# dotchen/LAV

Hardware: NVIDIA H100
Metric: agent_frames_per_s (higher is better)
Workload: dtype fp16 storage, fp32 accumulate (wgmma f16 / mma.sync f16; saturating stores)

## Files before the change

### include/lav_b200.h

```cpp
#ifndef LAV_B200_H
#define LAV_B200_H

#include <stddef.h>
#include <stdint.h>

#ifdef __cplusplus
extern "C" {
#endif

#define LAVB_ABI_VERSION 3

int lavb_abi_version(void);
const char* lavb_last_error(void);
int lavb_device_cc(void);

enum { LAVB_F32 = 0, LAVB_BF16 = 1, LAVB_F16 = 2 };
int lavb_h16_dtype(void);

int lavb_paint(const float* d_pts, int n, int pt_stride,
               const float* d_sem, int ncam, int c_in, int h, int w,
               long long s_cam, long long s_c, long long s_y, long long s_x,
               const float* h_cams, int mode,
               float* d_out, int out_stride, int out_col0, int copy_cols, void* stream);

// ... 115 lines not shown
int lavb_stack_job_poses(void* d_jobs, int b, int t, int gap, int keep, long long tick, double* d_ring_pose, const double* d_poses,
                         void* stream);

#define LAVB_VIEW_JET_ROWS 259
typedef struct lavb_view_config {
  double pixels_per_meter, cmd_thresh;
  unsigned char jet[LAVB_VIEW_JET_ROWS * 3];
} lavb_view_config;

size_t lavb_agent_view_scratch_bytes(int b);
int lavb_agent_view(const unsigned char* d_rgbs, const unsigned char* d_tels, const float* d_points, int b, long long p,
                    int point_stride, const void* d_bev, int bev_dtype, int bev_c, const long long* h_bev_strides, const float* d_plan,
                    const float* d_cast, const int* d_cmd, int t, const float* d_other_locs, const float* d_other_cmds, int k, int m,
                    const int* h_offsets, const double* h_boxes, int n_boxes, const int* h_box_offsets, const float* d_target,
                    const lavb_view_config* h_config, void* d_scratch, size_t scratch_bytes, unsigned char* d_out, void* stream);

size_t lavb_pillar_workspace_bytes(int batch, int nx, int ny);
int lavb_pillar_forward(const float* d_pts, int pt_stride, int d,
                        const long long* h_cloud_start, const int* h_cloud_count, int batch,
                        float min_x, float max_x, float min_y, float max_y, float ppm, int nx, int ny,
                        const float* d_w1, const float* d_s1, const float* d_t1, int h1,
                        const float* d_w2, const float* d_s2, const float* d_t2, int h2,
                        void* d_canvas, int canvas_dtype, void* d_workspace, void* stream);

size_t lavb_pillar_sorted_workspace_bytes(int batch, int nx, int ny, long long total_points);
int lavb_pillar_forward_sorted(const float* d_pts, int pt_stride, int d,
                               const long long* h_cloud_start, const int* h_cloud_count, int batch,
                               float min_x, float max_x, float min_y, float max_y, float ppm, int nx, int ny,
                               const float* d_w1, const float* d_s1, const float* d_t1, int h1,
                               const float* d_w2, const float* d_s2, const float* d_t2, int h2,
                               void* d_canvas, int out_mode, void* d_workspace, void* stream);

int lavb_pillar_decorate(const float* d_pts, int pt_stride, int d,
                         const long long* h_cloud_start, const int* h_cloud_count, int batch,
                         float min_x, float max_x, float min_y, float max_y, float ppm, int nx, int ny,
                         float* d_feat, int* d_cell, int* h_m, void* d_workspace, void* stream);
int lavb_pillar_scatter_max(const float* d_h, const int* d_cell, int m, int c, long long n_cells,
                            float* d_canvas, int* d_argmax, void* stream);
int lavb_pillar_scatter_max_bwd(const float* d_gcanvas, const int* d_argmax, const int* d_cell, int m, int c,
                                float* d_gh, void* stream);

typedef struct {
  const void* in; int in_dtype; int n, hin, win, cin, in_cstride, in_coff;
  void* out; int out_dtype; int hout, wout, cout, out_cstride, out_coff;
  int hog, wog;
  int in_sy, in_sx, out_sy, out_sx, out_oy, out_ox;
  int ntaps; int dy[16]; int dx[16];
  const float* w; const float* bias; const float* scale; const float* shift;
  const void* res; int res_dtype; int res_cstride, res_coff;
  int pre_relu, post_relu, sigmoid;
  int d2s_nout;
} lavb_conv_desc;
int lavb_conv_taps(const lavb_conv_desc* h_desc, void* stream);

int lavb_deconv3x3s2_small(const void* d_in, int dtype, int n, int h, int w, int in_cstride, int groups, int cin_g,
                           const float* d_w, const float* d_bias, const int* h_n_out, const int* h_sigmoid,
                           float* const* h_out_ptrs, void* stream);

int lavb_pool2_affine_relu(const void* d_in, int dtype, int n, int hin, int win, int c, int in_cstride, int in_coff,
                           const float* d_scale, const float* d_shift,
                           void* d_out, int out_cstride, int out_coff, void* stream);

int lavb_rgb_normalize(const void* d_rgb, int src_is_u8_nhwc, int n, int h, int w, void* d_out, int out_dtype,
                       void* stream);

int lavb_stem7x7s2_u8(const void* d_img, int batch, int ncam, int h, int cam_w, const void* d_w, const float* d_bias,
                      const float* h_mean, const float* h_std, void* d_out, void* stream);
int lavb_maxpool3x3s2_nhwc(const void* d_in, int n, int h, int w, int c, void* d_out, void* stream);

size_t lavb_det_peaks_workspace_bytes(int batch, int ncls);
int lavb_det_peaks(const float* d_center, const float* d_box, const float* d_ori, int batch, int h, int w, int ncls,
                   float min_score, int max_det, float* d_packed, void* d_workspace, void* stream);

int lavb_crop_bilinear(const void* d_feat, int dtype, int b, int h, int w, int c, const int* d_frame_idx,
                       const float* d_theta, int k, int crop, void* d_out, void* stream);
int lavb_crop_bilinear_u8(const uint8_t* d_map, int b, int c, int h, int w, const int* d_frame_idx, const float* d_theta,
                          int k, int crop, float* d_out, void* stream);
int lavb_crop_bilinear_bwd(const float* d_gout, int b, int h, int w, int c, const int* d_frame_idx, const float* d_theta,
                           int k, int crop, float* d_gfeat, void* stream);

int lavb_convert(const void* d_src, int src_dtype, void* d_dst, int dst_dtype, long long count, void* stream);

int lavb_conv_umma(const lavb_conv_desc* h_desc, void* stream);

int lavb_conv7x7s2_umma(const void* d_in, int n, int h, int w, int cin, const void* d_w, const float* d_bias, void* d_out,
                        void* stream);

int lavb_conv3x3_umma(const void* d_in, int n, int h, int w, int cin, int stride, const void* d_w, int cout, const float* d_bias,
                      const float* d_scale, const float* d_shift, int pre_relu, void* d_out, void* stream);

typedef struct lavb_conv_pair_desc {
  const void* in; void* out; const void* res;
  int n, h, w, c, dil, post_relu;
  const void* w1; const float* bias1;
  const void* w2; const float* shift2;
} lavb_conv_pair_desc;
int lavb_conv_pair_umma(const lavb_conv_pair_desc* h_desc, void* stream);
int lavb_conv_pair_set_trace(void* d_buf, int tiles_per_cta);

int lavb_erf_stem(const void* d_rgb_u8, int n, int h, int w, const float* h_w27x16, const float* h_scale16,
                  const float* h_shift16, void* d_out, int out_dtype, void* stream);

int lavb_erf_down16(const void* d_in, void* d_out, int n, int h, int w, const float* d_w9, const float* d_st, void* stream);

int lavb_erf_nb16(const void* d_in, void* d_out, int n, int h, int w, const float* d_w4, const float* d_st, void* stream);

int lavb_cast_gru(const float* d_embd, int n, const float* d_wih_t, const float* d_whh_t, const float* d_bih, const float* d_bhh,
                  const float* d_wmlp, const float* d_bmlp, int ncmd, int steps, float* d_out, void* stream);

#ifdef __cplusplus
}
#endif
#endif
```

### lav_b200/capi.py

```python
import ctypes as C
import os

_HERE = os.path.dirname(os.path.abspath(__file__))
LIB_PATH = os.path.join(_HERE, "_lib", "liblavb200.so")

F32, BF16, F16 = 0, 1, 2


class LavbError(RuntimeError):
    pass


class ConvDesc(C.Structure):
    _fields_ = [
        ("inp", C.c_void_p), ("in_dtype", C.c_int), ("n", C.c_int), ("hin", C.c_int), ("win", C.c_int), ("cin", C.c_int),
        ("in_cstride", C.c_int), ("in_coff", C.c_int),
        ("out", C.c_void_p), ("out_dtype", C.c_int), ("hout", C.c_int), ("wout", C.c_int), ("cout", C.c_int),
        ("out_cstride", C.c_int), ("out_coff", C.c_int),
        ("hog", C.c_int), ("wog", C.c_int),
        ("in_sy", C.c_int), ("in_sx", C.c_int), ("out_sy", C.c_int), ("out_sx", C.c_int), ("out_oy", C.c_int), ("out_ox", C.c_int),
        ("ntaps", C.c_int), ("dy", C.c_int * 16), ("dx", C.c_int * 16),
        ("w", C.c_void_p), ("bias", C.c_void_p), ("scale", C.c_void_p), ("shift", C.c_void_p),
        ("res", C.c_void_p), ("res_dtype", C.c_int), ("res_cstride", C.c_int), ("res_coff", C.c_int),
        ("pre_relu", C.c_int), ("post_relu", C.c_int), ("sigmoid", C.c_int), ("d2s_nout", C.c_int),
# ... 53 lines not shown
    "lavb_det_heatmaps": (C.c_int, [C.c_void_p, C.c_void_p, C.c_int, C.c_int, C.c_int, C.c_float, C.c_float, C.c_float, C.c_float,
                                    C.c_float, C.c_void_p, C.c_void_p, C.c_void_p, C.c_void_p]),
    "lavb_eval_batch": (C.c_int, [C.c_void_p, C.c_int, C.c_void_p, C.c_int, C.c_int, C.c_int, C.c_int, C.c_void_p, C.c_int,
                                  C.c_void_p, C.c_int, C.c_void_p, C.c_float, C.c_float, C.c_float, C.c_float, C.c_double,
                                  C.c_void_p, C.c_void_p, C.c_int, C.c_void_p, C.c_void_p, C.c_void_p, C.c_void_p, C.c_void_p,
                                  C.c_void_p]),
    "lavb_forecast_eval": (C.c_int, [C.c_void_p, C.c_void_p, C.c_void_p, C.c_void_p, C.c_int, C.c_int, C.c_int, C.c_void_p,
                                     C.c_void_p, C.c_void_p]),
    "lavb_det_forecast_match": (C.c_int, [C.c_void_p, C.c_int, C.c_int, C.c_int, C.c_void_p, C.c_int, C.c_void_p, C.c_void_p,
                                          C.c_void_p, C.c_void_p, C.c_void_p, C.c_void_p, C.c_int, C.c_int, C.c_float, C.c_float,
                                          C.c_float, C.c_float, C.c_double, C.c_void_p, C.c_void_p, C.c_void_p, C.c_void_p,
                                          C.c_void_p, C.c_void_p]),
    "lavb_det_box_eval": (C.c_int, [C.c_void_p, C.c_int, C.c_int, C.c_int, C.c_void_p, C.c_int, C.c_void_p, C.c_float, C.c_float,
                                    C.c_float, C.c_float, C.c_double, C.c_void_p, C.c_void_p, C.c_void_p, C.c_void_p, C.c_void_p,
                                    C.c_void_p]),
    "lavb_plan_safety": (C.c_int, [C.c_void_p, C.c_int, C.c_int, C.c_int, C.c_void_p, C.c_int, C.c_void_p, C.c_void_p, C.c_void_p,
                                   C.c_longlong, C.c_int, C.c_int, C.c_float, C.c_float, C.c_float, C.c_float, C.c_void_p,
                                   C.c_void_p]),
    "lavb_agent_control_state_bytes": (C.c_size_t, [C.c_int, C.c_int]),
    "lavb_agent_control": (C.c_int, [C.c_void_p, C.c_void_p, C.c_int, C.c_int, C.c_int, C.c_void_p, C.c_void_p, C.c_int, C.c_void_p,
                                     C.c_void_p, C.c_void_p, C.c_void_p, C.POINTER(ControlConfig), C.c_void_p, C.c_void_p,
                                     C.c_void_p, C.c_void_p]),
    "lavb_agent_control_dcmd": (C.c_int, [C.c_void_p, C.c_void_p, C.c_int, C.c_int, C.c_int, C.c_void_p, C.c_void_p, C.c_int,
                                          C.c_void_p, C.c_void_p, C.c_void_p, C.c_void_p, C.POINTER(ControlConfig), C.c_void_p,
                                          C.c_void_p, C.c_void_p, C.c_void_p]),
    "lavb_agent_nav_state_bytes": (C.c_size_t, []),
    "lavb_agent_nav_front": (C.c_int, [C.c_int, C.c_void_p, C.c_void_p, C.c_int, C.c_void_p, C.c_void_p, C.c_void_p, C.c_void_p,
                                       C.c_void_p, C.c_void_p, C.c_void_p, C.c_void_p, C.c_void_p]),
    "lavb_agent_nav_update": (C.c_int, [C.c_int, C.c_void_p, C.c_void_p, C.c_void_p, C.c_void_p, C.c_void_p, C.c_void_p]),
    "lavb_stack_job_poses": (C.c_int, [C.c_void_p, C.c_int, C.c_int, C.c_int, C.c_int, C.c_longlong, C.c_void_p, C.c_void_p,
                                       C.c_void_p]),
    "lavb_agent_view_scratch_bytes": (C.c_size_t, [C.c_int]),
    "lavb_agent_view": (C.c_int, [C.c_void_p, C.c_void_p, C.c_void_p, C.c_int, C.c_longlong, C.c_int, C.c_void_p, C.c_int, C.c_int,
                                  C.c_void_p, C.c_void_p, C.c_void_p, C.c_void_p, C.c_int, C.c_void_p, C.c_void_p, C.c_int, C.c_int,
                                  C.c_void_p, C.c_void_p, C.c_int, C.c_void_p, C.c_void_p, C.POINTER(ViewConfig), C.c_void_p,
                                  C.c_size_t, C.c_void_p, C.c_void_p]),
    "lavb_roof_filter": (C.c_int, [C.c_void_p, C.c_int, C.c_int, C.c_int, C.c_longlong, C.c_void_p, C.c_longlong, C.c_void_p, C.c_int,
                                   C.c_void_p]),
    "lavb_stack_sweep": (C.c_int, [C.c_void_p, C.c_int, C.c_int, C.c_void_p, C.c_float, C.c_float, C.c_int, C.c_int, C.c_int,
                                   C.c_void_p, C.c_void_p]),
    "lavb_pillar_workspace_bytes": (C.c_size_t, [C.c_int, C.c_int, C.c_int]),
    "lavb_pillar_forward": (C.c_int, [C.c_void_p, C.c_int, C.c_int, C.c_void_p, C.c_void_p, C.c_int,
                                      C.c_float, C.c_float, C.c_float, C.c_float, C.c_float, C.c_int, C.c_int,
                                      C.c_void_p, C.c_void_p, C.c_void_p, C.c_int, C.c_void_p, C.c_void_p, C.c_void_p, C.c_int,
                                      C.c_void_p, C.c_int, C.c_void_p, C.c_void_p]),
    "lavb_pillar_sorted_workspace_bytes": (C.c_size_t, [C.c_int, C.c_int, C.c_int, C.c_longlong]),
    "lavb_pillar_forward_sorted": (C.c_int, [C.c_void_p, C.c_int, C.c_int, C.c_void_p, C.c_void_p, C.c_int,
                                             C.c_float, C.c_float, C.c_float, C.c_float, C.c_float, C.c_int, C.c_int,
                                             C.c_void_p, C.c_void_p, C.c_void_p, C.c_int, C.c_void_p, C.c_void_p, C.c_void_p, C.c_int,
                                             C.c_void_p, C.c_int, C.c_void_p, C.c_void_p]),
    "lavb_pillar_decorate": (C.c_int, [C.c_void_p, C.c_int, C.c_int, C.c_void_p, C.c_void_p, C.c_int,
                                       C.c_float, C.c_float, C.c_float, C.c_float, C.c_float, C.c_int, C.c_int,
                                       C.c_void_p, C.c_void_p, C.c_void_p, C.c_void_p, C.c_void_p]),
    "lavb_pillar_scatter_max": (C.c_int, [C.c_void_p, C.c_void_p, C.c_int, C.c_int, C.c_longlong, C.c_void_p, C.c_void_p,
                                          C.c_void_p]),
    "lavb_pillar_scatter_max_bwd": (C.c_int, [C.c_void_p, C.c_void_p, C.c_void_p, C.c_int, C.c_int, C.c_void_p, C.c_void_p]),
    "lavb_conv_taps": (C.c_int, [C.POINTER(ConvDesc), C.c_void_p]),
    "lavb_pool2_affine_relu": (C.c_int, [C.c_void_p, C.c_int, C.c_int, C.c_int, C.c_int, C.c_int, C.c_int, C.c_int,
                                         C.c_void_p, C.c_void_p, C.c_void_p, C.c_int, C.c_int, C.c_void_p]),
    "lavb_rgb_normalize": (C.c_int, [C.c_void_p, C.c_int, C.c_int, C.c_int, C.c_int, C.c_void_p, C.c_int, C.c_void_p]),
    "lavb_convert": (C.c_int, [C.c_void_p, C.c_int, C.c_void_p, C.c_int, C.c_longlong, C.c_void_p]),
    "lavb_stem7x7s2_u8": (C.c_int, [C.c_void_p, C.c_int, C.c_int, C.c_int, C.c_int, C.c_void_p, C.c_void_p, C.c_void_p, C.c_void_p,
                                    C.c_void_p, C.c_void_p]),
    "lavb_erf_stem": (C.c_int, [C.c_void_p, C.c_int, C.c_int, C.c_int, C.c_void_p, C.c_void_p, C.c_void_p, C.c_void_p, C.c_int, C.c_void_p]),
    "lavb_erf_down16": (C.c_int, [C.c_void_p, C.c_void_p, C.c_int, C.c_int, C.c_int, C.c_void_p, C.c_void_p, C.c_void_p]),
    "lavb_erf_nb16": (C.c_int, [C.c_void_p, C.c_void_p, C.c_int, C.c_int, C.c_int, C.c_void_p, C.c_void_p, C.c_void_p]),
    "lavb_conv_pair_umma": (C.c_int, [C.c_void_p, C.c_void_p]),
    "lavb_maxpool3x3s2_nhwc": (C.c_int, [C.c_void_p, C.c_int, C.c_int, C.c_int, C.c_int, C.c_void_p, C.c_void_p]),
    "lavb_det_peaks_workspace_bytes": (C.c_size_t, [C.c_int, C.c_int]),
    "lavb_det_peaks": (C.c_int, [C.c_void_p, C.c_void_p, C.c_void_p, C.c_int, C.c_int, C.c_int, C.c_int, C.c_float, C.c_int,
                                 C.c_void_p, C.c_void_p, C.c_void_p]),
    "lavb_crop_bilinear": (C.c_int, [C.c_void_p, C.c_int, C.c_int, C.c_int, C.c_int, C.c_int, C.c_void_p, C.c_void_p, C.c_int,
                                     C.c_int, C.c_void_p, C.c_void_p]),
    "lavb_crop_bilinear_u8": (C.c_int, [C.c_void_p, C.c_int, C.c_int, C.c_int, C.c_int, C.c_void_p, C.c_void_p, C.c_int, C.c_int,
                                        C.c_void_p, C.c_void_p]),
    "lavb_cast_gru": (C.c_int, [C.c_void_p, C.c_int, C.c_void_p, C.c_void_p, C.c_void_p, C.c_void_p, C.c_void_p, C.c_void_p, C.c_int,
                                C.c_int, C.c_void_p, C.c_void_p]),
    "lavb_conv_pair_set_trace": (C.c_int, [C.c_void_p, C.c_int]),
    "lavb_crop_bilinear_bwd": (C.c_int, [C.c_void_p, C.c_int, C.c_int, C.c_int, C.c_int, C.c_void_p, C.c_void_p, C.c_int, C.c_int,
                                         C.c_void_p, C.c_void_p]),
    "lavb_deconv3x3s2_small": (C.c_int, [C.c_void_p, C.c_int, C.c_int, C.c_int, C.c_int, C.c_int, C.c_int, C.c_int, C.c_void_p,
                                         C.c_void_p, C.c_void_p, C.c_void_p, C.c_void_p, C.c_void_p]),
    "lavb_conv_umma": (C.c_int, [C.POINTER(ConvDesc), C.c_void_p]),
    "lavb_conv7x7s2_umma": (C.c_int, [C.c_void_p, C.c_int, C.c_int, C.c_int, C.c_int, C.c_void_p, C.c_void_p, C.c_void_p,
                                      C.c_void_p]),
    "lavb_conv3x3_umma": (C.c_int, [C.c_void_p, C.c_int, C.c_int, C.c_int, C.c_int, C.c_int, C.c_void_p, C.c_int, C.c_void_p,
                                    C.c_void_p, C.c_void_p, C.c_int, C.c_void_p, C.c_void_p]),
}

_lib = None


def exported_symbols():
    return sorted(_SIGS)


def lib():
    global _lib
    if _lib is None:
        if not os.path.exists(LIB_PATH):
            raise LavbError(f"{LIB_PATH} is missing — run `python -m lav_b200.build` (or __graft_entry__.build()); "
                            "lav_b200 has no CPU fallback")
        handle = C.CDLL(LIB_PATH)
        for name, (res, args) in _SIGS.items():
            fn = getattr(handle, name)
            fn.restype = res
            fn.argtypes = args
        if handle.lavb_abi_version() != 3:
            raise LavbError("liblavb200.so ABI version mismatch")
        _lib = handle
    return _lib


def h16_code():
    return lib().lavb_h16_dtype()


def check(code, what):
    if code != 0:
        raise LavbError(f"{what} failed ({code}): {lib().lavb_last_error().decode()}")
```

### lav_b200/csrc/conv_umma.cu

```cuda
#include "sm90.cuh"

namespace lavb {

constexpr int kTileH = 8, kTileW = 16, kBlockM = 128, kBlockK = 64;
constexpr int kABytes = kBlockM * kBlockK * 2;
constexpr int kMaxStages = 8;
constexpr int kMaxTaps = 16;
constexpr int kConvThreads = 288;

struct ConvArgs {
  int n, hog, wog, tiles_x, tiles_y, num_tiles;
  int hout, wout, cin, cout, kchunks, ntaps, stages;
  int in_sy, in_sx, out_sy, out_sx, out_oy, out_ox;
  int out_cstride, out_coff, out_is_f32, res_cstride, res_coff;
  int pre_bias, pre_relu, post_relu, sigmoid, d2s_nout, cout_store;
  int dy[kMaxTaps], dx[kMaxTaps];
  void* out; const h16* res;
  const float* bias; const float* scale; const float* shift;
};

using namespace sm90;

template <int kNC>
__global__ void __launch_bounds__(kConvThreads, kNC <= 4 ? 2 : 1) conv_umma_kernel(const __grid_constant__ CUtensorMap tmap_a,
                                                                                 const __grid_constant__ CUtensorMap tmap_b,
                                                                                 const __grid_constant__ ConvArgs p) {
  constexpr int kN = 32 * kNC;
  constexpr int kBBytes = kN * kBlockK * 2;
  constexpr int kStageBytes = kABytes + kBBytes;
  extern __shared__ uint8_t smem_raw[];
  const uint32_t base = (smem_u32(smem_raw) + 1023u) & ~1023u;
  uint8_t* gen = smem_raw + (base - smem_u32(smem_raw));
  const uint32_t ctrl = base + p.stages * kStageBytes;
  const uint32_t full_bar = ctrl, empty_bar = ctrl + 8 * kMaxStages;
  float* ep_bias = reinterpret_cast<float*>(gen + (ctrl - base) + 16 * kMaxStages);
  float* ep_st = ep_bias + 256;

  const int warp = threadIdx.x >> 5, lane = threadIdx.x & 31;
  if (threadIdx.x == 0) {
    asm volatile("prefetch.tensormap [%0];" ::"l"(reinterpret_cast<uint64_t>(&tmap_a)) : "memory");
    asm volatile("prefetch.tensormap [%0];" ::"l"(reinterpret_cast<uint64_t>(&tmap_b)) : "memory");
    for (int s = 0; s < p.stages; ++s) { mbar_init(full_bar + 8 * s, 1); mbar_init(empty_bar + 8 * s, 8); }
    asm volatile("fence.mbarrier_init.release.cluster;" ::: "memory");
  }
  for (int c = threadIdx.x; c < kN; c += blockDim.x) {
    const bool real = c < p.cout_store;
    const float b = (p.bias && real) ? __ldg(p.bias + c) : 0.f;
    const float sc = (p.scale && real) ? __ldg(p.scale + c) : 1.f;
    const float sh = (p.shift && real) ? __ldg(p.shift + c) : 0.f;
    ep_bias[c] = b;
    ep_st[2 * c] = sc;
    ep_st[2 * c + 1] = p.pre_bias ? sh : fmaf(b, sc, sh);
  }
  __syncthreads();
  const int nkb = p.ntaps * p.kchunks;
  const int tiles_per_img = p.tiles_x * p.tiles_y;

  if (warp == 8) {
    if (lane == 0) {
      int stage = 0; uint32_t phase = 0;
      for (int tile = blockIdx.x; tile < p.num_tiles; tile += gridDim.x) {
        const int img = tile / tiles_per_img, r = tile - img * tiles_per_img;
        const int y0 = (r / p.tiles_x) * kTileH * p.in_sy, x0 = (r % p.tiles_x) * kTileW * p.in_sx;
        for (int t = 0; t < p.ntaps; ++t) {
          for (int kc = 0; kc < p.kchunks; ++kc) {
            mbar_wait(empty_bar + 8 * stage, phase ^ 1);
            const uint32_t sa = base + stage * kStageBytes;
            mbar_expect_tx(full_bar + 8 * stage, kStageBytes);
            tma_load_4d(sa, &tmap_a, full_bar + 8 * stage, kc * kBlockK, x0 + p.dx[t], y0 + p.dy[t], img);
            tma_load_2d(sa + kABytes, &tmap_b, full_bar + 8 * stage, kc * kBlockK, t * kN);
            if (++stage == p.stages) { stage = 0; phase ^= 1; }
          }
        }
      }
    }
    return;
  }

  const int wg = warp >> 2;
  const float lo_pre = p.pre_relu ? 0.f : -INFINITY, lo_post = p.post_relu ? 0.f : -INFINITY;
  int stage = 0; uint32_t phase = 0;
  float acc[16 * kNC];
  for (int tile = blockIdx.x; tile < p.num_tiles; tile += gridDim.x) {
    int prev_stage = -1;
    for (int kb = 0; kb < nkb; ++kb) {
      mbar_wait(full_bar + 8 * stage, phase);
      const uint32_t sa = base + stage * kStageBytes;
      const uint64_t a_desc = sm90::desc_sw128(sa + wg * (kABytes / 2)), b_desc = sm90::desc_sw128(sa + kABytes);
      sm90::wgmma_fence();
#pragma unroll
      for (int k = 0; k < kBlockK / 16; ++k)
        sm90::wgmma<kN>(acc, a_desc + (uint64_t)(2 * k), b_desc + (uint64_t)(2 * k), (kb | k) ? 1u : 0u);
      sm90::wgmma_commit();
      sm90::wgmma_wait<1>();
      if (prev_stage >= 0 && lane == 0) mbar_arrive(empty_bar + 8 * prev_stage);
      prev_stage = stage;
      if (++stage == p.stages) { stage = 0; phase ^= 1; }
    }
    sm90::wgmma_wait<0>();
    sm90::acc_fence(acc);
    if (prev_stage >= 0 && lane == 0) mbar_arrive(empty_bar + 8 * prev_stage);

    const int c0 = 2 * (lane & 3), store_lim = p.cout_store - c0;
    const int img = tile / tiles_per_img, r = tile - img * tiles_per_img;
    const int gy = (r / p.tiles_x) * kTileH + 4 * wg + (warp & 3), oy = gy * p.out_sy + p.out_oy;
    if (!(gy < p.hog && oy < p.hout)) continue;
#pragma unroll
    for (int h = 0; h < 2; ++h) {
      const int gx = (r % p.tiles_x) * kTileW + (lane >> 2) + 8 * h, ox = gx * p.out_sx + p.out_ox;
      if (!(gx < p.wog && ox < p.wout)) continue;
      const long long pix = ((long long)img * p.hout + oy) * p.wout + ox;
      uint8_t* out_at = reinterpret_cast<uint8_t*>(p.out) + (pix * p.out_cstride + p.out_coff + c0) * (p.out_is_f32 ? 4 : 2);
      const h16* res_at = p.res ? p.res + pix * p.res_cstride + p.res_coff + c0 : nullptr;
      const float* bias_at = ep_bias + c0;
      const float* st_at = ep_st + 2 * c0;
#pragma unroll
      for (int j = 0; j < 4 * kNC; ++j) {
        const int g = 8 * j;
        float x0 = acc[4 * j + 2 * h], x1 = acc[4 * j + 2 * h + 1];
        if (p.pre_bias) { x0 += bias_at[g]; x1 += bias_at[g + 1]; }
        const float4 st = *reinterpret_cast<const float4*>(st_at + 2 * g);
        x0 = fmaf(fmaxf(x0, lo_pre), st.x, st.y);
        x1 = fmaf(fmaxf(x1, lo_pre), st.z, st.w);
        if (res_at) {
          const float2 rv = unpack_h16(__ldg(reinterpret_cast<const uint32_t*>(res_at + g)));
          x0 += rv.x; x1 += rv.y;
        }
        x0 = fmaxf(x0, lo_post); x1 = fmaxf(x1, lo_post);
        if (p.sigmoid) { x0 = 1.f / (1.f + expf(-x0)); x1 = 1.f / (1.f + expf(-x1)); }
        if (kNC == 1 && p.d2s_nout) {
          float* ob = reinterpret_cast<float*>(p.out);
          const int no = p.d2s_nout;
#pragma unroll
          for (int e = 0; e < 2; ++e) {
            const int q = g + c0 + e;
            if (q < 4 * no) {
              const int pos = q / no, k = q - pos * no;
              ob[(pix + (long long)(pos >> 1) * p.wout + (pos & 1)) * no + k] = e ? x1 : x0;
            }
          }
        } else if (g < store_lim) {
          if (p.out_is_f32)
            *reinterpret_cast<float2*>(out_at + 4 * g) = make_float2(x0, x1);
          else
            *reinterpret_cast<uint32_t*>(out_at + 2 * g) = pack_h16(x0, x1);
        }
      }
    }
  }
}

}

using namespace lavb;

extern "C" int lavb_conv_umma(const lavb_conv_desc* d, void* stream) {
  LAVB_CHECK_ARG(d != nullptr, "conv_umma: null descriptor");
  LAVB_CHECK_ARG(d->in_dtype == LAVB_H16, "conv_umma: input must be h16");
  LAVB_CHECK_ARG(d->out_dtype == LAVB_H16 || d->out_dtype == LAVB_F32, "conv_umma: bad output dtype");
  LAVB_CHECK_ARG(d->ntaps >= 1 && d->ntaps <= kMaxTaps, "conv_umma: ntaps must be 1..16");
  LAVB_CHECK_ARG(d->cin % 64 == 0 && d->cin > 0, "conv_umma: cin must be a multiple of 64 (got %d)", d->cin);
  LAVB_CHECK_ARG(d->cout % 8 == 0 && d->cout >= 8 && d->cout <= 256, "conv_umma: cout must be 8..256, multiple of 8 (got %d)", d->cout);
  const int cout_mma = (d->cout + 31) / 32 * 32;
  LAVB_CHECK_ARG(d->res == nullptr || cout_mma == d->cout, "conv_umma: residual needs cout %% 32 == 0");
  LAVB_CHECK_ARG(d->in_cstride % 8 == 0 && d->in_coff % 8 == 0 && d->in_coff + d->cin <= d->in_cstride, "conv_umma: input slice misaligned");
  LAVB_CHECK_ARG(d->out_cstride % 8 == 0 && d->out_coff % 8 == 0 && d->out_coff + d->cout <= d->out_cstride, "conv_umma: output slice misaligned");
  LAVB_CHECK_ARG(d->res == nullptr || (d->res_dtype == LAVB_H16 && d->res_cstride % 8 == 0 && d->res_coff % 8 == 0), "conv_umma: residual must be h16, 16 B aligned");
  LAVB_CHECK_ARG((d->scale == nullptr) == (d->shift == nullptr), "conv_umma: scale and shift come together");
  LAVB_CHECK_ARG(d->in_sy >= 1 && d->in_sy <= 8 && d->in_sx >= 1 && d->in_sx <= 8, "conv_umma: bad input stride");
  auto encode = get_encode();
  LAVB_CHECK_ARG(encode != nullptr, "conv_umma: cuTensorMapEncodeTiled not available from the driver");

  CUtensorMap tmap_a, tmap_b;
  {
    const h16* in = reinterpret_cast<const h16*>(d->in) + d->in_coff;
    cuuint64_t dims[4] = {(cuuint64_t)d->cin, (cuuint64_t)d->win, (cuuint64_t)d->hin, (cuuint64_t)d->n};
    cuuint64_t strides[3] = {(cuuint64_t)d->in_cstride * 2, (cuuint64_t)d->win * d->in_cstride * 2,
                             (cuuint64_t)d->hin * d->win * d->in_cstride * 2};
    cuuint32_t box[4] = {(cuuint32_t)kBlockK, (cuuint32_t)(kTileW * d->in_sx), (cuuint32_t)(kTileH * d->in_sy), 1};
    cuuint32_t estr[4] = {1, (cuuint32_t)d->in_sx, (cuuint32_t)d->in_sy, 1};
    CUresult r = encode(&tmap_a, LAVB_TMAP_H16, 4, const_cast<h16*>(in), dims, strides, box, estr,
                        CU_TENSOR_MAP_INTERLEAVE_NONE, CU_TENSOR_MAP_SWIZZLE_128B, CU_TENSOR_MAP_L2_PROMOTION_L2_256B,
                        CU_TENSOR_MAP_FLOAT_OOB_FILL_NONE);
    LAVB_CHECK_ARG(r == CUDA_SUCCESS, "conv_umma: cuTensorMapEncodeTiled(A) failed with %d", (int)r);
  }
  {
    cuuint64_t dims[2] = {(cuuint64_t)d->cin, (cuuint64_t)d->ntaps * cout_mma};
    cuuint64_t strides[1] = {(cuuint64_t)d->cin * 2};
    cuuint32_t box[2] = {(cuuint32_t)kBlockK, (cuuint32_t)cout_mma};
    cuuint32_t estr[2] = {1, 1};
    CUresult r = encode(&tmap_b, LAVB_TMAP_H16, 2, const_cast<float*>(d->w), dims, strides, box, estr,
                        CU_TENSOR_MAP_INTERLEAVE_NONE, CU_TENSOR_MAP_SWIZZLE_128B, CU_TENSOR_MAP_L2_PROMOTION_L2_256B,
                        CU_TENSOR_MAP_FLOAT_OOB_FILL_NONE);
    LAVB_CHECK_ARG(r == CUDA_SUCCESS, "conv_umma: cuTensorMapEncodeTiled(B) failed with %d", (int)r);
  }
  ConvArgs a;
  memset(&a, 0, sizeof(a));
  a.n = d->n; a.hog = d->hog; a.wog = d->wog;
  a.tiles_x = ceil_div(d->wog, kTileW); a.tiles_y = ceil_div(d->hog, kTileH);
  a.num_tiles = a.n * a.tiles_x * a.tiles_y;
  a.hout = d->hout; a.wout = d->wout; a.cin = d->cin; a.cout = cout_mma; a.cout_store = d->cout; a.kchunks = d->cin / kBlockK;
  a.ntaps = d->ntaps;
  const int nc = cout_mma / 32;
  const bool two_per_sm = nc <= 4;
  const int stage_bytes = kABytes + cout_mma * kBlockK * 2;
  const int ctrl_bytes = 1024  + 16 * kMaxStages + 3 * 256 * (int)sizeof(float);
  const int smem_cap = two_per_sm ? 113 * 1024 : 227 * 1024;
  a.stages = min(kMaxStages, (smem_cap - ctrl_bytes) / stage_bytes);
  a.in_sy = d->in_sy; a.in_sx = d->in_sx; a.out_sy = d->out_sy; a.out_sx = d->out_sx; a.out_oy = d->out_oy; a.out_ox = d->out_ox;
  a.out_cstride = d->out_cstride; a.out_coff = d->out_coff; a.out_is_f32 = d->out_dtype == LAVB_F32;
  a.res_cstride = d->res_cstride; a.res_coff = d->res_coff;
  a.pre_bias = d->pre_relu && d->bias != nullptr;
  a.pre_relu = d->pre_relu; a.post_relu = d->post_relu; a.sigmoid = d->sigmoid; a.d2s_nout = d->d2s_nout;
  if (d->d2s_nout) {
    LAVB_CHECK_ARG(d->cout == 32 && d->d2s_nout >= 1 && 4 * d->d2s_nout <= 32 && d->out_dtype == LAVB_F32 && d->out_sy == 2 &&
                   d->out_sx == 2 && d->res == nullptr, "conv_umma: depth-to-space epilogue needs cout=32, fp32 out, out_s=2, no residual");
  }
  for (int t = 0; t < d->ntaps; ++t) { a.dy[t] = d->dy[t]; a.dx[t] = d->dx[t]; }
  a.out = d->out; a.res = reinterpret_cast<const h16*>(d->res);
  a.bias = d->bias; a.scale = d->scale; a.shift = d->shift;
  if (a.num_tiles == 0) return 0;
  const int smem = a.stages * stage_bytes + ctrl_bytes;
  const int grid = min(a.num_tiles, two_per_sm ? 2 * kNumSMs : kNumSMs);
#define LAVB_CONV_LAUNCH(NC)                                                                                              \
  case NC: {                                                                                                              \
                             \
    LAVB_CUDA_OK(ensure_dyn_smem((const void*)conv_umma_kernel<NC>, smem_cap));                                          \
    conv_umma_kernel<NC><<<grid, kConvThreads, smem, (cudaStream_t)stream>>>(tmap_a, tmap_b, a);                          \
    break;                                                                                                                \
  }
  switch (nc) {
    LAVB_CONV_LAUNCH(1) LAVB_CONV_LAUNCH(2) LAVB_CONV_LAUNCH(3) LAVB_CONV_LAUNCH(4)
    LAVB_CONV_LAUNCH(5) LAVB_CONV_LAUNCH(6) LAVB_CONV_LAUNCH(7) LAVB_CONV_LAUNCH(8)
  }
#undef LAVB_CONV_LAUNCH
  LAVB_LAUNCH_OK();
  return 0;
}
```

### lav_b200/layers.py

```python
import torch

from . import ops

USE_UMMA = True
UMMA_STRIDED = True


def bn_affine(bn, eps=None):
    eps = bn.eps if eps is None else eps
    var = bn.running_var.double()
    scale = bn.weight.double() / torch.sqrt(var + eps)
    shift = bn.bias.double() - bn.running_mean.double() * scale
    return scale.float().contiguous(), shift.float().contiguous()


def _pad_cout(w_tco):
    t, ci, co = w_tco.shape
    cp = (co + 15) // 16 * 16
    out = torch.zeros((t, ci, cp), dtype=torch.float32, device=w_tco.device)
    out[:, :, :co] = w_tco
    return out.contiguous()


def cmajor_wins(hout, wout):
    return hout >= 80 and wout >= 80


class TapConv:
    def __init__(self, weight, transposed=False, stride=1, padding=0, dilation=1, output_padding=0, bias=None,
                 pre_relu=False, scale=None, shift=None, post_relu=False, sigmoid=False, cin_pad=None):
        pair = lambda v: (v, v) if isinstance(v, int) else tuple(v)
        self.stride, self.padding, self.dilation, self.opad = pair(stride), pair(padding), pair(dilation), pair(output_padding)
        self.transposed = transposed
        w = weight.detach().float()
        if transposed:
            self.cin, self.cout, self.kh, self.kw = w.shape
        else:
            self.cout, self.cin, self.kh, self.kw = w.shape
        self.cin_k = cin_pad or self.cin
        self.bias = bias.detach().float().contiguous() if bias is not None else None
        self.scale = scale.contiguous() if scale is not None else None
        self.shift = shift.contiguous() if shift is not None else None
        self.pre_relu, self.post_relu, self.sigmoid = pre_relu, post_relu, sigmoid
        sy, sx = self.stride
        py_, px_ = self.padding
        dy_, dx_ = self.dilation
        self.phases = []
        if not transposed:
            taps, blocks = [], []
            for ky in range(self.kh):
                for kx in range(self.kw):
                    taps.append((ky * dy_ - py_, kx * dx_ - px_))
                    blocks.append(self._block(w[:, :, ky, kx].t()))
            self.phases.append(dict(taps=taps, w=_pad_cout(torch.stack(blocks)), in_s=(sy, sx), out_s=(1, 1), out_o=(0, 0)))
        else:
            for oy in range(sy):
                for ox in range(sx):
                    taps, blocks = [], []
                    for ky in range(self.kh):
                        if (oy + py_ - ky * dy_) % sy:
                            continue
                        for kx in range(self.kw):
                            if (ox + px_ - kx * dx_) % sx:
                                continue
                            taps.append(((oy + py_ - ky * dy_) // sy, (ox + px_ - kx * dx_) // sx))
                            blocks.append(self._block(w[:, :, ky, kx]))
                    if not taps:
                        taps, blocks = [(0, 0)], [torch.zeros((self.cin_k, self.cout), device=w.device)]
                    self.phases.append(dict(taps=taps, w=_pad_cout(torch.stack(blocks)), in_s=(1, 1), out_s=(sy, sx),
                                            out_o=(oy, ox)))
        for ph in self.phases:
            assert len(ph["taps"]) <= 16, "tap list longer than the kernel's table"
        self.umma_ok = USE_UMMA and self.cin_k % 64 == 0 and self.cout % 8 == 0 and self.cout <= 256
        self.cmajor_ok = (self.umma_ok and not transposed and (self.kh, self.kw) == (3, 3) and self.padding == (1, 1)
                          and self.dilation == (1, 1) and self.stride in ((1, 1), (2, 2)) and self.cin_k in (64, 128, 384)
                          and self.cout in (64, 128, 256) and not post_relu and not sigmoid)
        if self.umma_ok:
            cm = (self.cout + 31) // 32 * 32
            for ph in self.phases:
                wu = torch.zeros((len(ph["taps"]), cm, self.cin_k), dtype=ops.h16(), device=ph["w"].device)
                wu[:, :self.cout] = ph["w"][:, :, :self.cout].permute(0, 2, 1).to(ops.h16())
                ph["w_umma"] = wu.contiguous()

    def _block(self, w_ci_co):
        if self.cin_k == self.cin:
            return w_ci_co
        out = torch.zeros((self.cin_k, self.cout), dtype=w_ci_co.dtype, device=w_ci_co.device)
        out[:self.cin] = w_ci_co
        return out

    def out_size(self, hin, win):
        (sy, sx), (py_, px_), (dy_, dx_), (oy, ox) = self.stride, self.padding, self.dilation, self.opad
        if self.transposed:
            return ((hin - 1) * sy - 2 * py_ + dy_ * (self.kh - 1) + oy + 1, (win - 1) * sx - 2 * px_ + dx_ * (self.kw - 1) + ox + 1)
        return ((hin + 2 * py_ - dy_ * (self.kh - 1) - 1) // sy + 1, (win + 2 * px_ - dx_ * (self.kw - 1) - 1) // sx + 1)

    def __call__(self, x, out=None, in_coff=0, out_coff=0, out_channels=None, res=None, res_coff=0, out_dtype=None):
        n, hin, win, _ = x.shape
        hout, wout = self.out_size(hin, win)
        if out is None:
            out = torch.empty((n, hout, wout, out_channels or self.cout), dtype=out_dtype or x.dtype, device=x.device)
        if (self.cmajor_ok and cmajor_wins(hout, wout) and x.dtype == ops.h16()
                and out.dtype == ops.h16() and x.shape[3] == self.cin_k and in_coff == 0 and out.shape[3] == self.cout
                and out_coff == 0 and res is None):
            ph = self.phases[0]
            return ops.conv3x3_umma(x, ph["w_umma"], self.cout, self.stride[0], self.bias, self.scale, self.shift, self.pre_relu,
                                    out=out)
        for ph in self.phases:
            osy, osx = ph["out_s"]
            ooy, oox = ph["out_o"]
            hog, wog = (hout - ooy + osy - 1) // osy, (wout - oox + osx - 1) // osx
            umma = (self.umma_ok and x.dtype == ops.h16() and (res is None or (res.dtype == ops.h16() and self.cout % 32 == 0))
                    and (UMMA_STRIDED or ph["in_s"] == (1, 1)))
            ops.conv_taps(x, self.cin_k, in_coff, out, self.cout, out_coff, hog, wog, ph["in_s"], ph["out_s"], ph["out_o"],
                          ph["taps"], ph["w_umma"] if umma else ph["w"], self.bias, self.scale, self.shift, res, res_coff,
                          self.pre_relu, self.post_relu, self.sigmoid, umma=umma)
        return out


class PlanMixin:

    def _plan_get(self, device, builder):
        plans = self.__dict__.setdefault("_lavb_plans", {})
        key = (str(device), getattr(self, "precision", "fp32"))
        if key not in plans:
            with torch.no_grad():
                plans[key] = builder(device)
        return plans[key]

    def invalidate_plan(self):
        for m in self.modules():
            if isinstance(m, PlanMixin):
                m.__dict__["_lavb_plans"] = {}

    def _apply(self, fn, *a, **k):
        self.__dict__["_lavb_plans"] = {}
        return super()._apply(fn, *a, **k)

    def load_state_dict(self, *a, **k):
        self.invalidate_plan()
        return super().load_state_dict(*a, **k)

    def train(self, mode=True):
        self.__dict__["_lavb_plans"] = {}
        return super().train(mode)
```

### lav_b200/ops.py

```python
import ctypes as C
import math

import numpy as np
import torch

from . import capi
from .capi import BF16, F16, F32, ConvDesc, check, lib

_DT = {torch.float32: F32, torch.bfloat16: BF16, torch.float16: F16}


def h16():
    return torch.float16 if capi.h16_code() == F16 else torch.bfloat16



def _stream():
    return C.c_void_p(torch.cuda.current_stream().cuda_stream)


def _ptr(t):
    return C.c_void_p(t.data_ptr()) if t is not None else C.c_void_p(0)


# ... 101 lines not shown
        out = torch.empty_like(x)
    _tensor("roof_filter", "out", out, None, x.shape)
    _require(out.data_ptr() != x.data_ptr(), "roof_filter: out must not be the sweeps' storage")
    counts = torch.empty((f,), dtype=torch.int32, device=x.device)
    _launch("lavb_roof_filter", _ptr(x), f, n, cols, n * cols, _ptr(out), n * cols, _ptr(counts), int(pad_nan))
    return (out if sweeps.dim() == 3 else out[0]), counts


def _workspace(device, nbytes):
    return torch.empty(int(nbytes), dtype=torch.uint8, device=device)


def _clouds(starts, counts, pts, what):
    b = len(counts)
    starts, counts = [int(s) for s in starts], [int(c) for c in counts]
    if len(starts) != b:
        raise capi.LavbError(f"{what}: {len(starts)} starts for {b} counts")
    for i, (s, c) in enumerate(zip(starts, counts)):
        if c > 0 and s + c > pts.shape[0]:
            raise capi.LavbError(f"{what}: cloud {i} = rows [{s}, {s + c}) lies past the {pts.shape[0]} rows of pts")
    st = (C.c_longlong * b)(*starts)
    ct = (C.c_int * b)(*counts)
    return b, st, ct


_POINT_MLP = (("w1", (64, 16)), ("s1", (64,)), ("t1", (64,)), ("w2", (64, 64)), ("s2", (64,)), ("t2", (64,)))


def pillar_forward(pts, starts, counts, grid, w1, s1, t1, w2, s2, t2):
    _tensor("pillar_forward", "pts", pts, torch.float32, (None, None), contiguous=False)
    _require(pts.stride(1) == 1 and pts.shape[1] >= 11, f"pillar_forward: point rows must be unit-stride and hold at least 11 "
             f"floats, got {tuple(pts.shape)} with strides {pts.stride()}")
    for (name, shape), t in zip(_POINT_MLP, (w1, s1, t1, w2, s2, t2)):
        _tensor("pillar_forward", name, t, torch.float32, shape, pts.device)
    min_x, max_x, min_y, max_y, ppm, nx, ny = grid
    d = w1.shape[1] - 5
    b, st, ct = _clouds(starts, counts, pts, "pillar_forward")
    canvas = torch.empty((b, ny, nx, w2.shape[0]), dtype=torch.float32, device=pts.device)
    ws = _workspace(pts.device, lib().lavb_pillar_workspace_bytes(b, nx, ny))
    _launch("lavb_pillar_forward", _ptr(pts), pts.stride(0), d, st, ct, b, min_x, max_x, min_y, max_y, ppm, nx, ny, _ptr(w1),
            _ptr(s1), _ptr(t1), w1.shape[0], _ptr(w2), _ptr(s2), _ptr(t2), w2.shape[0], _ptr(canvas), F32, _ptr(ws), launches=4,
            prof=("pillar", float(sum(int(c) for c in counts)) * d * 4 + canvas.numel() * 4))
    return canvas


def pillar_decorate(pts, starts, counts, grid, d):
    _tensor("pillar_decorate", "pts", pts, torch.float32, (None, None), contiguous=False)
    _require(pts.stride(1) == 1, "pillar_decorate: pts must have unit stride along a row")
    min_x, max_x, min_y, max_y, ppm, nx, ny = grid
    b, st, ct = _clouds(starts, counts, pts, "pillar_decorate")
    ws = _workspace(pts.device, lib().lavb_pillar_workspace_bytes(b, nx, ny))
    total = int(sum(int(c) for c in counts))
    feat = torch.empty((total, d + 5), dtype=torch.float32, device=pts.device)
    cell = torch.empty((total,), dtype=torch.int32, device=pts.device)
    m = C.c_int(0)
    _launch("lavb_pillar_decorate", _ptr(pts), pts.stride(0), d, st, ct, b, min_x, max_x, min_y, max_y, ppm, nx, ny, _ptr(feat),
            _ptr(cell), C.byref(m), _ptr(ws), launches=4)
    return feat[:m.value], cell[:m.value]


def pillar_scatter_max(h, cell, n_cells, want_argmax=True):
    m, c = _tensor("pillar_scatter_max", "h", h, torch.float32, (None, None), contiguous=False)
    _tensor("pillar_scatter_max", "cell", cell, torch.int32, (m,), h.device)
    _require(int(n_cells) >= 0, f"pillar_scatter_max: n_cells = {n_cells} < 0")
    h = h.contiguous()
    canvas = torch.empty((n_cells, c), dtype=torch.float32, device=h.device)
    arg = torch.empty((n_cells, c), dtype=torch.int32, device=h.device) if want_argmax else None
    _launch("lavb_pillar_scatter_max", _ptr(h), _ptr(cell), m, c, n_cells, _ptr(canvas), _ptr(arg), launches=2)
    return canvas, arg


def pillar_scatter_max_bwd(gcanvas, arg, cell, m):
    shape = _tensor("pillar_scatter_max_bwd", "gcanvas", gcanvas, torch.float32, (None, None), contiguous=False)
    _tensor("pillar_scatter_max_bwd", "arg", arg, torch.int32, shape, gcanvas.device)
    _tensor("pillar_scatter_max_bwd", "cell", cell, torch.int32, (m,), gcanvas.device)
    gcanvas = gcanvas.contiguous()
    c = gcanvas.shape[-1]
    gh = torch.empty((m, c), dtype=torch.float32, device=gcanvas.device)
    _launch("lavb_pillar_scatter_max_bwd", _ptr(gcanvas), _ptr(arg), _ptr(cell), m, c, _ptr(gh))
    return gh


def conv_taps(x, cin, in_coff, out, cout, out_coff, hog, wog, in_s, out_s, out_o, taps, w, bias=None, scale=None, shift=None,
              res=None, res_coff=0, pre_relu=False, post_relu=False, sigmoid=False, umma=False, d2s_nout=0):
    _tensor("conv_taps", "x", x, h16() if umma else None, (None,) * 4)
    _tensor("conv_taps", "out", out, torch.float32 if d2s_nout else None, (x.shape[0], None, None, d2s_nout or None))
    _tensor("conv_taps", "w", w, h16() if umma else torch.float32,
            (len(taps), (cout + 31) // 32 * 32, cin) if umma else (len(taps), cin, (cout + 15) // 16 * 16))
    _require(not d2s_nout or (umma and cout == 32 and 4 * d2s_nout <= 32),
             f"conv_taps: d2s_nout = {d2s_nout} needs the wgmma kernel, cout 32 and 4 * d2s_nout <= 32")
    d = ConvDesc()
    d.inp, d.in_dtype = x.data_ptr(), _DT[x.dtype]
    d.n, d.hin, d.win, d.in_cstride = x.shape
    d.cin, d.in_coff = cin, in_coff
    d.out, d.out_dtype = out.data_ptr(), _DT[out.dtype]
    _, d.hout, d.wout, d.out_cstride = out.shape
    d.cout, d.out_coff = cout, out_coff
    d.d2s_nout = d2s_nout
    if d2s_nout:
        d.out_cstride, d.out_coff = 32, 0
    d.hog, d.wog = hog, wog
    d.in_sy, d.in_sx = in_s
    d.out_sy, d.out_sx = out_s
    d.out_oy, d.out_ox = out_o
    d.ntaps = len(taps)
    for i, (dy, dx) in enumerate(taps):
        d.dy[i], d.dx[i] = dy, dx
    d.w = w.data_ptr()
    d.bias = bias.data_ptr() if bias is not None else None
    d.scale = scale.data_ptr() if scale is not None else None
    d.shift = shift.data_ptr() if shift is not None else None
    if res is not None:
        _tensor("conv_taps", "res", res, None, (*out.shape[:3], None))
        d.res, d.res_dtype, d.res_cstride, d.res_coff = res.data_ptr(), _DT[res.dtype], res.shape[3], res_coff
    d.pre_relu, d.post_relu, d.sigmoid = int(pre_relu), int(post_relu), int(sigmoid)
    _launch("lavb_conv_umma" if umma else "lavb_conv_taps", C.byref(d),
            prof=(f"umma:{cin}->{cout}x{len(taps)}taps@{hog}x{wog}", 2.0 * x.shape[0] * hog * wog * cout * cin * len(taps))
            if umma else None)
    return out


def pool2_affine_relu(x, c, in_coff, scale, shift, out, out_coff):
    _need_cuda(x, out)
    n, h, w, cs = x.shape
    _launch("lavb_pool2_affine_relu", _ptr(x), _DT[x.dtype], n, h, w, c, cs, in_coff, _ptr(scale), _ptr(shift), _ptr(out),
            out.shape[3], out_coff)
    return out


def rgb_normalize(rgb, out_dtype=torch.float32):
    if torch.is_tensor(rgb) and rgb.dtype == torch.uint8:
        n, h, w, _ = _tensor("rgb_normalize", "rgb", rgb, None, (None, None, None, 3), contiguous=False)
        rgb, u8 = rgb.contiguous(), 1
    else:
        n, _, h, w = _tensor("rgb_normalize", "rgb", rgb, None, (None, 3, None, None), contiguous=False)
        rgb, u8 = rgb.float().contiguous(), 0
    out = torch.empty((n, h, w, 4), dtype=out_dtype, device=rgb.device)
    _launch("lavb_rgb_normalize", _ptr(rgb), u8, n, h, w, _ptr(out), _DT[out_dtype])
    return out


def convert(src, dtype):
    _need_cuda(src)
    src = src.contiguous()
    if src.dtype == dtype:
        return src
    dst = torch.empty(src.shape, dtype=dtype, device=src.device)
    _launch("lavb_convert", _ptr(src), _DT[src.dtype], _ptr(dst), _DT[dtype], src.numel())
    return dst


def crop_supported(feats_nhwc):
    vec = {torch.float32: 4, h16(): 8}.get(feats_nhwc.dtype)
    return (vec is not None and feats_nhwc.dim() == 4 and feats_nhwc.is_contiguous() and feats_nhwc.data_ptr() % 16 == 0
            and feats_nhwc.shape[3] > 0 and feats_nhwc.shape[3] % vec == 0)


def _crop_poses(what, frame_idx, theta, b):
    k, _, _ = _tensor(what, "theta", theta, None, (None, 2, 3), contiguous=False)
    _tensor(what, "frame_idx", frame_idx, None, (k,), contiguous=False)
    _require(not (frame_idx.dtype.is_floating_point or frame_idx.dtype.is_complex or frame_idx.dtype == torch.bool),
             f"{what}: frame_idx must be an integer tensor, got {frame_idx.dtype}")
    if frame_idx.dtype != torch.int32:
        frame_idx = frame_idx.clamp(0, b - 1).to(torch.int32)
    return k, frame_idx.contiguous(), theta.float().contiguous()


def crop_bilinear(feats_nhwc, frame_idx, theta, crop_size):
    _need_cuda(feats_nhwc)
    _require(crop_supported(feats_nhwc), f"crop_bilinear: need a contiguous, 16-byte aligned (B,H,W,C) map, fp32 with C % 4 == 0 "
             f"or {h16()} with C % 8 == 0; got {feats_nhwc.dtype} {tuple(feats_nhwc.shape)}")
    b, h, w, c = feats_nhwc.shape
    k, frame_idx, theta = _crop_poses("crop_bilinear", frame_idx, theta, b)
    out = torch.empty((k, crop_size, crop_size, c), dtype=feats_nhwc.dtype, device=feats_nhwc.device)
    _launch("lavb_crop_bilinear", _ptr(feats_nhwc), _DT[feats_nhwc.dtype], b, h, w, c, _ptr(frame_idx), _ptr(theta), k, crop_size,
            _ptr(out))
    return out


def crop_bilinear_u8(bev_u8, frame_idx, theta, crop_size, out=None):
    _need_cuda(frame_idx)
    b, c, h, w = _tensor("crop_bilinear_u8", "bev_u8", bev_u8, torch.uint8, (None,) * 4)
    k, _, _ = _tensor("crop_bilinear_u8", "theta", theta, None, (None, 2, 3), contiguous=False)
    _require(frame_idx.numel() == k, f"crop_bilinear_u8: frame_idx {tuple(frame_idx.shape)} does not hold one frame per crop (K = {k})")
    theta = theta.float().contiguous()
    frame_idx = frame_idx.to(torch.int32).contiguous()
    out = _out("crop_bilinear_u8", "out", out, torch.float32, (k, c, crop_size, crop_size), bev_u8.device)
    _launch("lavb_crop_bilinear_u8", _ptr(bev_u8), b, c, h, w, _ptr(frame_idx), _ptr(theta), k, crop_size, _ptr(out))
    return out


def crop_bilinear_bwd(gout_nhwc, frame_idx, theta, feat_shape, out=None):
    _require(len(feat_shape) == 4, f"crop_bilinear_bwd: feat_shape must be (B, H, W, C), got {tuple(feat_shape)}")
    b, h, w, c = (int(v) for v in feat_shape)
    _tensor("crop_bilinear_bwd", "gout", gout_nhwc, torch.float32, (None,) * 4)
    _require(gout_nhwc.data_ptr() % 16 == 0, "crop_bilinear_bwd: gout must be 16-byte aligned")
    k, frame_idx, theta = _crop_poses("crop_bilinear_bwd", frame_idx, theta, b)
    crop = gout_nhwc.shape[1]
# ... 701 lines not shown
```

Measured before the change: 2097.

## Run all sub-pixel phases of a strided/transposed conv in one wgmma launch

Adds a phase table to the wgmma conv kernel so that each tile index also selects a phase, with its own tap range and output offset. Multi-phase convolutions (transposed or strided decompositions) now issue one launch over the concatenated taps and weights instead of one launch per phase. This is meant to cut launch overhead and fill the GPU better with more tiles per grid. In exchange it adds per-tile integer divides and a larger kernel argument struct.

```diff
diff --git a/include/lav_b200.h b/include/lav_b200.h
--- a/include/lav_b200.h
+++ b/include/lav_b200.h
@@ -221,6 +221,8 @@
 int lavb_convert(const void* d_src, int src_dtype, void* d_dst, int dst_dtype, long long count, void* stream);
 
 int lavb_conv_umma(const lavb_conv_desc* h_desc, void* stream);
+int lavb_conv_umma_phases(const lavb_conv_desc* h_desc, int nphase, const int* h_ntaps, const int* h_oy, const int* h_ox,
+                          void* stream);
 
 int lavb_conv7x7s2_umma(const void* d_in, int n, int h, int w, int cin, const void* d_w, const float* d_bias, void* d_out,
                         void* stream);
diff --git a/lav_b200/capi.py b/lav_b200/capi.py
--- a/lav_b200/capi.py
+++ b/lav_b200/capi.py
@@ -159,6 +159,8 @@
     "lavb_deconv3x3s2_small": (C.c_int, [C.c_void_p, C.c_int, C.c_int, C.c_int, C.c_int, C.c_int, C.c_int, C.c_int, C.c_void_p,
                                          C.c_void_p, C.c_void_p, C.c_void_p, C.c_void_p, C.c_void_p]),
     "lavb_conv_umma": (C.c_int, [C.POINTER(ConvDesc), C.c_void_p]),
+    "lavb_conv_umma_phases": (C.c_int, [C.POINTER(ConvDesc), C.c_int, C.POINTER(C.c_int), C.POINTER(C.c_int),
+                                        C.POINTER(C.c_int), C.c_void_p]),
     "lavb_conv7x7s2_umma": (C.c_int, [C.c_void_p, C.c_int, C.c_int, C.c_int, C.c_int, C.c_void_p, C.c_void_p, C.c_void_p,
                                       C.c_void_p]),
     "lavb_conv3x3_umma": (C.c_int, [C.c_void_p, C.c_int, C.c_int, C.c_int, C.c_int, C.c_int, C.c_void_p, C.c_int, C.c_void_p,
diff --git a/lav_b200/csrc/conv_umma.cu b/lav_b200/csrc/conv_umma.cu
--- a/lav_b200/csrc/conv_umma.cu
+++ b/lav_b200/csrc/conv_umma.cu
@@ -15,6 +15,7 @@
   int out_cstride, out_coff, out_is_f32, res_cstride, res_coff;
   int pre_bias, pre_relu, post_relu, sigmoid, d2s_nout, cout_store;
   int dy[kMaxTaps], dx[kMaxTaps];
+  int nphase, ph_tap0[kMaxTaps], ph_ntaps[kMaxTaps], ph_oy[kMaxTaps], ph_ox[kMaxTaps];
   void* out; const h16* res;
   const float* bias; const float* scale; const float* shift;
 };
@@ -53,16 +54,16 @@
     ep_st[2 * c + 1] = p.pre_bias ? sh : fmaf(b, sc, sh);
   }
   __syncthreads();
-  const int nkb = p.ntaps * p.kchunks;
   const int tiles_per_img = p.tiles_x * p.tiles_y;
 
   if (warp == 8) {
     if (lane == 0) {
       int stage = 0; uint32_t phase = 0;
       for (int tile = blockIdx.x; tile < p.num_tiles; tile += gridDim.x) {
-        const int img = tile / tiles_per_img, r = tile - img * tiles_per_img;
+        const int pt = tile / p.nphase, f = tile - pt * p.nphase;
+        const int img = pt / tiles_per_img, r = pt - img * tiles_per_img;
         const int y0 = (r / p.tiles_x) * kTileH * p.in_sy, x0 = (r % p.tiles_x) * kTileW * p.in_sx;
-        for (int t = 0; t < p.ntaps; ++t) {
+        for (int t = p.ph_tap0[f]; t < p.ph_tap0[f] + p.ph_ntaps[f]; ++t) {
           for (int kc = 0; kc < p.kchunks; ++kc) {
             mbar_wait(empty_bar + 8 * stage, phase ^ 1);
             const uint32_t sa = base + stage * kStageBytes;
@@ -83,6 +84,8 @@
   float acc[16 * kNC];
   for (int tile = blockIdx.x; tile < p.num_tiles; tile += gridDim.x) {
     int prev_stage = -1;
+    const int pt = tile / p.nphase, f = tile - pt * p.nphase;
+    const int nkb = p.ph_ntaps[f] * p.kchunks;
     for (int kb = 0; kb < nkb; ++kb) {
       mbar_wait(full_bar + 8 * stage, phase);
       const uint32_t sa = base + stage * kStageBytes;
@@ -102,12 +105,12 @@
     if (prev_stage >= 0 && lane == 0) mbar_arrive(empty_bar + 8 * prev_stage);
 
     const int c0 = 2 * (lane & 3), store_lim = p.cout_store - c0;
-    const int img = tile / tiles_per_img, r = tile - img * tiles_per_img;
-    const int gy = (r / p.tiles_x) * kTileH + 4 * wg + (warp & 3), oy = gy * p.out_sy + p.out_oy;
+    const int img = pt / tiles_per_img, r = pt - img * tiles_per_img;
+    const int gy = (r / p.tiles_x) * kTileH + 4 * wg + (warp & 3), oy = gy * p.out_sy + p.ph_oy[f];
     if (!(gy < p.hog && oy < p.hout)) continue;
 #pragma unroll
     for (int h = 0; h < 2; ++h) {
-      const int gx = (r % p.tiles_x) * kTileW + (lane >> 2) + 8 * h, ox = gx * p.out_sx + p.out_ox;
+      const int gx = (r % p.tiles_x) * kTileW + (lane >> 2) + 8 * h, ox = gx * p.out_sx + p.ph_ox[f];
       if (!(gx < p.wog && ox < p.wout)) continue;
       const long long pix = ((long long)img * p.hout + oy) * p.wout + ox;
       uint8_t* out_at = reinterpret_cast<uint8_t*>(p.out) + (pix * p.out_cstride + p.out_coff + c0) * (p.out_is_f32 ? 4 : 2);
@@ -154,8 +157,8 @@
 
 using namespace lavb;
 
-extern "C" int lavb_conv_umma(const lavb_conv_desc* d, void* stream) {
-  LAVB_CHECK_ARG(d != nullptr, "conv_umma: null descriptor");
+static int conv_umma_launch(const lavb_conv_desc* d, int nphase, const int* ph_ntaps, const int* ph_oy, const int* ph_ox,
+                            void* stream) {
   LAVB_CHECK_ARG(d->in_dtype == LAVB_H16, "conv_umma: input must be h16");
   LAVB_CHECK_ARG(d->out_dtype == LAVB_H16 || d->out_dtype == LAVB_F32, "conv_umma: bad output dtype");
   LAVB_CHECK_ARG(d->ntaps >= 1 && d->ntaps <= kMaxTaps, "conv_umma: ntaps must be 1..16");
@@ -198,7 +201,15 @@
   memset(&a, 0, sizeof(a));
   a.n = d->n; a.hog = d->hog; a.wog = d->wog;
   a.tiles_x = ceil_div(d->wog, kTileW); a.tiles_y = ceil_div(d->hog, kTileH);
-  a.num_tiles = a.n * a.tiles_x * a.tiles_y;
+  if (nphase == 0) {
+    a.nphase = 1; a.ph_tap0[0] = 0; a.ph_ntaps[0] = d->ntaps; a.ph_oy[0] = d->out_oy; a.ph_ox[0] = d->out_ox;
+  } else {
+    a.nphase = nphase;
+    for (int f = 0, t0 = 0; f < nphase; t0 += ph_ntaps[f++]) {
+      a.ph_tap0[f] = t0; a.ph_ntaps[f] = ph_ntaps[f]; a.ph_oy[f] = ph_oy[f]; a.ph_ox[f] = ph_ox[f];
+    }
+  }
+  a.num_tiles = a.n * a.tiles_x * a.tiles_y * a.nphase;
   a.hout = d->hout; a.wout = d->wout; a.cin = d->cin; a.cout = cout_mma; a.cout_store = d->cout; a.kchunks = d->cin / kBlockK;
   a.ntaps = d->ntaps;
   const int nc = cout_mma / 32;
@@ -237,3 +248,25 @@
   LAVB_LAUNCH_OK();
   return 0;
 }
+
+extern "C" int lavb_conv_umma(const lavb_conv_desc* d, void* stream) {
+  LAVB_CHECK_ARG(d != nullptr, "conv_umma: null descriptor");
+  return conv_umma_launch(d, 0, nullptr, nullptr, nullptr, stream);
+}
+
+extern "C" int lavb_conv_umma_phases(const lavb_conv_desc* d, int nphase, const int* h_ntaps, const int* h_oy, const int* h_ox,
+                                     void* stream) {
+  LAVB_CHECK_ARG(d != nullptr, "conv_umma_phases: null descriptor");
+  LAVB_CHECK_ARG(nphase >= 1 && nphase <= kMaxTaps, "conv_umma_phases: nphase must be 1..16 (got %d)", nphase);
+  LAVB_CHECK_ARG(h_ntaps != nullptr && h_oy != nullptr && h_ox != nullptr, "conv_umma_phases: null phase table");
+  LAVB_CHECK_ARG(d->out_sy >= 1 && d->out_sx >= 1, "conv_umma_phases: bad output stride");
+  LAVB_CHECK_ARG(d->d2s_nout == 0, "conv_umma_phases: no depth-to-space epilogue");
+  int total = 0;
+  for (int f = 0; f < nphase; ++f) {
+    LAVB_CHECK_ARG(h_ntaps[f] >= 1 && h_oy[f] >= 0 && h_ox[f] >= 0, "conv_umma_phases: phase %d needs ntaps >= 1, out_o >= 0", f);
+    total += h_ntaps[f];
+    LAVB_CHECK_ARG(total <= d->ntaps, "conv_umma_phases: the phases hold more taps than d->ntaps");
+  }
+  LAVB_CHECK_ARG(total == d->ntaps, "conv_umma_phases: the phases hold %d taps, d->ntaps is %d", total, d->ntaps);
+  return conv_umma_launch(d, nphase, h_ntaps, h_oy, h_ox, stream);
+}
diff --git a/lav_b200/layers.py b/lav_b200/layers.py
--- a/lav_b200/layers.py
+++ b/lav_b200/layers.py
@@ -4,6 +4,7 @@
 
 USE_UMMA = True
 UMMA_STRIDED = True
+UMMA_ONE_LAUNCH = True
 
 
 def bn_affine(bn, eps=None):
@@ -72,6 +73,7 @@
         for ph in self.phases:
             assert len(ph["taps"]) <= 16, "tap list longer than the kernel's table"
         self.umma_ok = USE_UMMA and self.cin_k % 64 == 0 and self.cout % 8 == 0 and self.cout <= 256
+        self.grouped = None
         self.cmajor_ok = (self.umma_ok and not transposed and (self.kh, self.kw) == (3, 3) and self.padding == (1, 1)
                           and self.dilation == (1, 1) and self.stride in ((1, 1), (2, 2)) and self.cin_k in (64, 128, 384)
                           and self.cout in (64, 128, 256) and not post_relu and not sigmoid)
@@ -81,6 +83,10 @@
                 wu = torch.zeros((len(ph["taps"]), cm, self.cin_k), dtype=ops.h16(), device=ph["w"].device)
                 wu[:, :self.cout] = ph["w"][:, :, :self.cout].permute(0, 2, 1).to(ops.h16())
                 ph["w_umma"] = wu.contiguous()
+            if len(self.phases) > 1 and sum(len(ph["taps"]) for ph in self.phases) <= 16:
+                self.grouped = dict(taps=[t for ph in self.phases for t in ph["taps"]],
+                                    w=torch.cat([ph["w_umma"] for ph in self.phases]).contiguous(),
+                                    phases=[(len(ph["taps"]), *ph["out_o"]) for ph in self.phases])
 
     def _block(self, w_ci_co):
         if self.cin_k == self.cin:
@@ -106,6 +112,13 @@
             ph = self.phases[0]
             return ops.conv3x3_umma(x, ph["w_umma"], self.cout, self.stride[0], self.bias, self.scale, self.shift, self.pre_relu,
                                     out=out)
+        if (UMMA_ONE_LAUNCH and self.grouped is not None and x.dtype == ops.h16()
+                and (res is None or (res.dtype == ops.h16() and self.cout % 32 == 0))):
+            g, (osy, osx) = self.grouped, self.phases[0]["out_s"]
+            ops.conv_taps(x, self.cin_k, in_coff, out, self.cout, out_coff, -(-hout // osy), -(-wout // osx), (1, 1),
+                          (osy, osx), (0, 0), g["taps"], g["w"], self.bias, self.scale, self.shift, res, res_coff,
+                          self.pre_relu, self.post_relu, self.sigmoid, umma=True, phases=g["phases"])
+            return out
         for ph in self.phases:
             osy, osx = ph["out_s"]
             ooy, oox = ph["out_o"]
diff --git a/lav_b200/ops.py b/lav_b200/ops.py
--- a/lav_b200/ops.py
+++ b/lav_b200/ops.py
@@ -207,13 +207,15 @@
 
 
 def conv_taps(x, cin, in_coff, out, cout, out_coff, hog, wog, in_s, out_s, out_o, taps, w, bias=None, scale=None, shift=None,
-              res=None, res_coff=0, pre_relu=False, post_relu=False, sigmoid=False, umma=False, d2s_nout=0):
+              res=None, res_coff=0, pre_relu=False, post_relu=False, sigmoid=False, umma=False, d2s_nout=0, phases=None):
     _tensor("conv_taps", "x", x, h16() if umma else None, (None,) * 4)
     _tensor("conv_taps", "out", out, torch.float32 if d2s_nout else None, (x.shape[0], None, None, d2s_nout or None))
     _tensor("conv_taps", "w", w, h16() if umma else torch.float32,
             (len(taps), (cout + 31) // 32 * 32, cin) if umma else (len(taps), cin, (cout + 15) // 16 * 16))
     _require(not d2s_nout or (umma and cout == 32 and 4 * d2s_nout <= 32),
              f"conv_taps: d2s_nout = {d2s_nout} needs the wgmma kernel, cout 32 and 4 * d2s_nout <= 32")
+    _require(phases is None or (umma and not d2s_nout and 1 <= len(phases) <= 16),
+             f"conv_taps: phases need the wgmma kernel, no d2s_nout and 1..16 entries")
     d = ConvDesc()
     d.inp, d.in_dtype = x.data_ptr(), _DT[x.dtype]
     d.n, d.hin, d.win, d.in_cstride = x.shape
@@ -239,6 +241,14 @@
         _tensor("conv_taps", "res", res, None, (*out.shape[:3], None))
         d.res, d.res_dtype, d.res_cstride, d.res_coff = res.data_ptr(), _DT[res.dtype], res.shape[3], res_coff
     d.pre_relu, d.post_relu, d.sigmoid = int(pre_relu), int(post_relu), int(sigmoid)
+    if phases is not None:
+        (osy, osx), (_, hout, wout, _) = out_s, out.shape
+        flop = sum(2.0 * x.shape[0] * ((hout - oy + osy - 1) // osy) * ((wout - ox + osx - 1) // osx) * cout * cin * nt
+                   for nt, oy, ox in phases)
+        tab = [(C.c_int * len(phases))(*v) for v in zip(*phases)]
+        _launch("lavb_conv_umma_phases", C.byref(d), len(phases), *tab,
+                prof=(f"umma:{cin}->{cout}x{len(taps)}taps/{len(phases)}phases@{hog}x{wog}", flop))
+        return out
     _launch("lavb_conv_umma" if umma else "lavb_conv_taps", C.byref(d),
             prof=(f"umma:{cin}->{cout}x{len(taps)}taps@{hog}x{wog}", 2.0 * x.shape[0] * hog * wog * cout * cin * len(taps))
             if umma else None)
```

New measurement: 2100, median of 6. About the same (+0.2%).
